# jdwapman/essentials

Hardware: NVIDIA B200
Metric: BFS GTEPS (higher is better)
Workload: dtype int32

## Files before the change

### essentials_b200/csrc/capi_core.cu

```cuda
#include "capi_common.hxx"
#include <algorithm>
#include <memory>
#include <gunrock/algorithms/generate/random.hxx>
#include <gunrock/algorithms/sssp.hxx>

namespace ess {
std::string& last_error() {
  static thread_local std::string message;
  return message;
}
int fail(const std::exception& e) {
  last_error() = e.what();
  return 999;
}
int fail(const char* message, int code) {
  last_error() = message;
  return code;
}
}

using namespace gunrock;

namespace ess {
int& dist_peer_exchange() {
  static int on = 1;
  return on;
}
int& dist_trace() {
  static int on = 0;
  return on;
}
int& dist_peer_timeout_ms() {
  static int ms = 4000;
  return ms;
}
int& host_chunk_edges() {
  static int edges = 64 << 20;
  return edges;
}
}

extern "C" {

const char* ess_last_error(void) { return ess::last_error().c_str(); }
int ess_version(void) { return 100; }

int ess_context_create(int device, void* stream, int own_stream, ess_context_t* out) {
  ESS_TRY
  if (!out) return ess::fail("ess_context_create: out is null");
  int count = 0;
  error::throw_if_exception(cudaGetDeviceCount(&count), "no CUDA device");
  error::throw_if_exception(device < 0 || device >= count, "ess_context_create: bad device ordinal");
  auto* h = new ess_context_s;
  if (own_stream)
    h->ctx = std::make_shared<gcuda::multi_context_t>(device);
  else
    h->ctx = std::make_shared<gcuda::multi_context_t>(device, static_cast<cudaStream_t>(stream));
  h->single()->scratch();
  *out = h;
  return 0;
  ESS_CATCH
}

int ess_context_destroy(ess_context_t ctx) {
  delete ctx;
  return 0;
}

int ess_context_synchronize(ess_context_t ctx) {
  ESS_TRY
  ctx->single()->synchronize();
  return 0;
  ESS_CATCH
}

int ess_tune(const char* knob, int value) {
  ESS_TRY
  const std::string k = knob ? knob : "";
  if (k == "near_far_ctas") {
    gunrock::operators::advance::near_far_ctas_per_sm() = value < 1 ? 1 : value;
    return 0;
  }
  if (k == "advance_engine") {
    gunrock::operators::advance::kernels::advance_engine() = value;
    return 0;
  }
  if (k == "pull_engine") {
    gunrock::operators::advance::kernels::pull_engine() = value;
    return 0;
  }
  if (k == "near_far_cluster") {
    gunrock::operators::advance::near_far_cluster_enabled() = value;
    return 0;
  }
  if (k == "pull_hints") {
    gunrock::operators::advance::kernels::pull_hints_enabled() = value;
    return 0;
  }
  if (k == "sssp_fused_unique") {
    gunrock::sssp::fused_unique() = value;
    return 0;
  }
  if (k == "dist_trace") {
    ess::dist_trace() = value;
    return 0;
  }
  if (k == "dist_peer_exchange") {
    ess::dist_peer_exchange() = value;
    return 0;
  }
  if (k == "host_chunk_edges") {
    if (value <= 0) return ess::fail("ess_tune: host_chunk_edges must be positive");
    ess::host_chunk_edges() = value;
    return 0;
  }
  if (k == "dist_peer_timeout_ms") {
    if (value <= 0) return ess::fail("ess_tune: dist_peer_timeout_ms must be positive");
    ess::dist_peer_timeout_ms() = value;
    return 0;
  }
  return ess::fail("ess_tune: unknown knob");
  ESS_CATCH
}

int ess_profile_enable(ess_context_t ctx, int enable) {
  ESS_TRY
  auto& prof = ctx->single()->profiler();
  prof.reset();
  prof.enabled = enable != 0;
  return 0;
  ESS_CATCH
}

int ess_profile_read(ess_context_t ctx, double* ms_by_class, int64_t* launches_by_class, int n_classes) {
  ESS_TRY
  auto& prof = ctx->single()->profiler();
  prof.collect();
  for (int i = 0; i < n_classes && i < gcuda::profiler_t::n_classes; ++i) {
    if (ms_by_class) ms_by_class[i] = prof.ms[i];
    if (launches_by_class) launches_by_class[i] = prof.launches[i];
  }
  if (launches_by_class && n_classes >= gcuda::profiler_t::n_classes)
    launches_by_class[gcuda::profiler_t::n_classes - 1] = prof.launches_total;
  return 0;
  ESS_CATCH
}

int ess_graph_create(int64_t n, int64_t m, int offset_bits, const void* d_row_offsets,
                     const int32_t* d_column_indices, const float* d_values, int symmetric,
                     const void* d_column_offsets, const int32_t* d_row_indices, const float* d_csc_values,
                     ess_graph_t* out) {
  ESS_TRY
  if (!out || !d_row_offsets || (m > 0 && !d_column_indices)) return ess::fail("ess_graph_create: null argument");
  if (offset_bits != 32 && offset_bits != 64) return ess::fail("ess_graph_create: offset_bits must be 32 or 64");
  if (n < 0 || n > 2147483647LL) return ess::fail("ess_graph_create: vertex ids are int32");
  if (offset_bits == 32 && m > 2147483647LL) return ess::fail("ess_graph_create: m needs 64-bit offsets");
  auto* h = new ess_graph_s;
  h->offset_bits = offset_bits;
  h->n = n;
  h->m = m;
  const void* t_off = d_column_offsets;
  const int32_t* t_idx = d_row_indices;
  const float* t_val = d_csc_values;
  if (symmetric) {
    t_off = d_row_offsets;
    t_idx = d_column_indices;
    t_val = d_values;
  }
  h->has_csc = t_off != nullptr;
  auto* J = const_cast<int32_t*>(d_column_indices);
  auto* X = const_cast<float*>(d_values);
  auto* I = const_cast<int32_t*>(t_idx);
  auto* Xt = const_cast<float*>(t_val);
  if (offset_bits == 64)
    h->g64 = graph::build::from_csr_and_csc<int32_t, int64_t, float>(
        int32_t(n), int64_t(m), (int64_t*)d_row_offsets, J, X, (int64_t*)t_off, I, Xt);
  else
    h->g32 = graph::build::from_csr_and_csc<int32_t, int32_t, float>(
        int32_t(n), int32_t(m), (int32_t*)d_row_offsets, J, X, (int32_t*)t_off, I, Xt);
  if (h->has_csc && symmetric != 2 && n > 0 && m > 0) {
    int rc = ess_graph_build_pull_hints(h, nullptr);
    if (rc) {
      delete h;
      return rc;
    }
  }
  *out = h;
  return 0;
  ESS_CATCH
}

}

namespace {
struct copy_lane_t {
  cudaStream_t stream = nullptr;
  std::vector<cudaEvent_t> events;
  copy_lane_t() { error::throw_if_exception(cudaStreamCreateWithFlags(&stream, cudaStreamNonBlocking), "copy stream"); }
  ~copy_lane_t() {
    for (auto e : events) cudaEventDestroy(e);
    if (stream) cudaStreamDestroy(stream);
  }
  void publish_to(cudaStream_t follower) {
    cudaEvent_t e = nullptr;
    error::throw_if_exception(cudaEventCreateWithFlags(&e, cudaEventDisableTiming), "copy event");
    events.push_back(e);
    error::throw_if_exception(cudaEventRecord(e, stream), "copy event record");
    error::throw_if_exception(cudaStreamWaitEvent(follower, e, 0), "copy event wait");
  }
};

template <typename edge_t>
void create_from_host(ess_context_t ctx, ess_graph_s* h, const void* h_row_offsets, const int32_t* h_column_indices,
                      const float* h_values, bool symmetric) {
  auto* c = ctx->single();
  cudaStream_t work = c->stream();
  const std::size_t n = std::size_t(h->n), m = std::size_t(h->m);
  const edge_t* ho = static_cast<const edge_t*>(h_row_offsets);
  error::throw_if_exception(ho[0] != edge_t(0) || std::size_t(ho[n]) != m,
                            "ess_graph_create_from_host: row_offsets[0] must be 0 and row_offsets[n] must be m");
  h->own_offsets.resize((n + 1) * sizeof(edge_t));
  h->own_indices.resize(m);
  if (h_values) h->own_values.resize(m);
  edge_t* d_off = reinterpret_cast<edge_t*>(h->own_offsets.data());
  int32_t* d_idx = h->own_indices.data();
  float* d_val = h_values ? h->own_values.data() : nullptr;

  copy_lane_t lane;
  error::throw_if_exception(cudaMemcpyAsync(d_off, ho, (n + 1) * sizeof(edge_t), cudaMemcpyHostToDevice, lane.stream),
                            "ess_graph_create_from_host: offsets copy");
  lane.publish_to(work);
  const bool hints = symmetric && n > 0 && m > 0;
  memory::device_array_t<int32_t> degree;
  edge_t* hint_edge = nullptr;
  if (hints) {
    h->hint_head.resize(n);
    h->hint_isolated.resize((n + 31) / 32 + 1);
    if constexpr (sizeof(edge_t) == 8) {
      h->hint_edge64.resize(n);
      hint_edge = h->hint_edge64.data();
    } else {
      h->hint_edge32.resize(n);
      hint_edge = h->hint_edge32.data();
    }
    degree.resize(n);
    graph::build::detail::degrees_kernel<<<2048, 256, 0, work>>>(int32_t(n), d_off, degree.data());
    graph::build::detail::isolated_bitmap_kernel<<<2048, 256, 0, work>>>(int32_t(n), d_off, h->hint_isolated.data());
  }
  const std::size_t chunk_edges = std::size_t(ess::host_chunk_edges());
  std::size_t built = 0;
  for (std::size_t e0 = 0; e0 < m; e0 += chunk_edges) {
    const std::size_t e1 = std::min(m, e0 + chunk_edges);
    error::throw_if_exception(cudaMemcpyAsync(d_idx + e0, h_column_indices + e0, (e1 - e0) * sizeof(int32_t),
                                              cudaMemcpyHostToDevice, lane.stream),
                              "ess_graph_create_from_host: indices copy");
    if (!hints) continue;
    lane.publish_to(work);
    const std::size_t arrived = std::size_t(std::upper_bound(ho, ho + n + 1, edge_t(e1)) - ho) - 1;
    graph::build::pull_hints_range(int32_t(built), int32_t(arrived), d_off, d_idx, degree.data(), h->hint_head.data(),
                                   hint_edge, work);
    built = std::max(built, arrived);
  }
  if (d_val)
    error::throw_if_exception(cudaMemcpyAsync(d_val, h_values, m * sizeof(float), cudaMemcpyHostToDevice, lane.stream),
                              "ess_graph_create_from_host: values copy");
  error::throw_if_exception(cudaStreamSynchronize(lane.stream), "ess_graph_create_from_host: copy");
  error::throw_if_exception(cudaStreamSynchronize(work), "ess_graph_create_from_host: hint build");
  error::check_last("ess_graph_create_from_host");

  auto G = graph::build::from_csr_and_csc<int32_t, edge_t, float>(int32_t(n), edge_t(m), d_off, d_idx, d_val,
                                                                  symmetric ? d_off : nullptr,
                                                                  symmetric ? d_idx : nullptr,
                                                                  symmetric ? d_val : nullptr);
  if (hints) {
    graph::graph_csc_t<int32_t, edge_t, float>& csc = G;
    csc.set_pull_hints(h->hint_head.data(), hint_edge, h->hint_isolated.data());
  }
  if constexpr (sizeof(edge_t) == 8)
    h->g64 = G;
  else
    h->g32 = G;
}
}

extern "C" {

int ess_graph_create_from_host(ess_context_t ctx, int64_t n, int64_t m, int offset_bits, const void* h_row_offsets,
                               const int32_t* h_column_indices, const float* h_values, int symmetric,
                               ess_graph_t* out) {
  ESS_TRY
  if (!ctx || !out || !h_row_offsets || (m > 0 && !h_column_indices))
    return ess::fail("ess_graph_create_from_host: null argument");
  if (offset_bits != 32 && offset_bits != 64)
    return ess::fail("ess_graph_create_from_host: offset_bits must be 32 or 64");
  if (n < 0 || n > 2147483647LL) return ess::fail("ess_graph_create_from_host: vertex ids are int32");
  if (m < 0 || (offset_bits == 32 && m > 2147483647LL))
    return ess::fail("ess_graph_create_from_host: m needs 64-bit offsets");
  std::unique_ptr<ess_graph_s> h(new ess_graph_s);
  h->offset_bits = offset_bits;
  h->n = n;
  h->m = m;
  h->has_csc = symmetric != 0;
  if (offset_bits == 64)
    create_from_host<int64_t>(ctx, h.get(), h_row_offsets, h_column_indices, h_values, symmetric != 0);
  else
    create_from_host<int32_t>(ctx, h.get(), h_row_offsets, h_column_indices, h_values, symmetric != 0);
  *out = h.release();
  return 0;
  ESS_CATCH
}

int ess_graph_build_pull_hints(ess_graph_t h, const int32_t* d_degree_of_id) {
  ESS_TRY
  if (!h || !h->has_csc) return ess::fail("ess_graph_build_pull_hints: graph has no CSC view");
  if (h->n <= 0 || h->m <= 0) return 0;
  error::throw_if_exception(cudaDeviceSynchronize(), "ess_graph_build_pull_hints: pending work failed");
  h->hint_head.resize(std::size_t(h->n));
  h->hint_isolated.resize((std::size_t(h->n) + 31) / 32 + 1);
  if (h->offset_bits == 64) {
    h->hint_edge64.resize(std::size_t(h->n));
    graph::build::pull_hints(h->g64, h->hint_head.data(), h->hint_edge64.data(), 0, d_degree_of_id,
                             h->hint_isolated.data());
  } else {
    h->hint_edge32.resize(std::size_t(h->n));
    graph::build::pull_hints(h->g32, h->hint_head.data(), h->hint_edge32.data(), 0, d_degree_of_id,
                             h->hint_isolated.data());
  }
  return 0;
  ESS_CATCH
}

int ess_graph_destroy(ess_graph_t g) {
  delete g;
  return 0;
}

int ess_transpose_csr(int64_t n, int64_t m, int offset_bits, const void* d_row_offsets,
                      const int32_t* d_column_indices, const float* d_values, void* d_out_offsets,
                      int32_t* d_out_indices, float* d_out_values) {
  ESS_TRY
  error::throw_if_exception(cudaDeviceSynchronize(), "ess_transpose_csr: pending work failed");
  if (offset_bits == 64)
    graph::build::detail::transpose_on_device<int32_t, int64_t, float>(
        int32_t(n), int64_t(m), (const int64_t*)d_row_offsets, d_column_indices, d_values, d_out_indices,
        (int64_t*)d_out_offsets, d_out_values);
  else
    graph::build::detail::transpose_on_device<int32_t, int32_t, float>(
        int32_t(n), int32_t(m), (const int32_t*)d_row_offsets, d_column_indices, d_values, d_out_indices,
        (int32_t*)d_out_offsets, d_out_values);
  return 0;
  ESS_CATCH
}

int ess_randoms(ess_context_t ctx, float* d_out, int64_t n, float begin, float end) {
  ESS_TRY
  generate::random::uniform_distribution(d_out, std::size_t(n), begin, end, ctx->single()->stream());
  error::check_last("ess_randoms");
  ctx->single()->synchronize();
  return 0;
  ESS_CATCH
}

int ess_frontier_to_bitmap(ess_context_t ctx, const int32_t* d_list, int64_t size, int64_t universe,
                           uint32_t* d_words, int64_t* popcount) {
  ESS_TRY
  auto* c = ctx->single();
  auto stream = c->stream();
  auto& scratch = c->scratch();
  const std::size_t words = (std::size_t(universe) + 31) / 32;
  cudaMemsetAsync(d_words, 0, words * sizeof(uint32_t), stream);
  if (size)
    frontier::kernels::scatter_bits_kernel<<<gcuda::persistent_grid(*c, (std::size_t(size) + 255) / 256, 8), 256, 0,
                                             stream>>>(d_list, std::size_t(size), d_words);
  scratch.zero(stream);
  frontier::kernels::popcount_kernel<<<gcuda::persistent_grid(*c, (words + 255) / 256, 8), 256, 0, stream>>>(
      d_words, words, scratch.d + gcuda::scratch_t::out_count);
  error::check_last("ess_frontier_to_bitmap");
  scratch.fetch(stream);
  if (popcount) *popcount = int64_t(scratch.h[gcuda::scratch_t::out_count]);
  return 0;
  ESS_CATCH
}

int ess_bitmap_to_frontier(ess_context_t ctx, const uint32_t* d_words, int64_t universe, int32_t* d_list,
                           int64_t* out_count) {
  ESS_TRY
  auto* c = ctx->single();
  auto stream = c->stream();
  auto& scratch = c->scratch();
  const std::size_t words = (std::size_t(universe) + 31) / 32;
  scratch.zero(stream);
  frontier::kernels::gather_bits_kernel<<<gcuda::persistent_grid(*c, (words + 255) / 256, 8), 256, 0, stream>>>(
      d_words, words, d_list, scratch.d + gcuda::scratch_t::out_count);
  error::check_last("ess_bitmap_to_frontier");
  scratch.fetch(stream);
  if (out_count) *out_count = int64_t(scratch.h[gcuda::scratch_t::out_count]);
  return 0;
  ESS_CATCH
}

int ess_bits_to_list_async(ess_context_t ctx, const uint32_t* d_words, int64_t universe, int32_t* d_list) {
  ESS_TRY
  auto* c = ctx->single();
  auto stream = c->stream();
  auto& scratch = c->scratch();
  const std::size_t words = (std::size_t(universe) + 31) / 32;
  scratch.zero(stream);
  frontier::kernels::gather_bits_kernel<<<gcuda::persistent_grid(*c, (words + 255) / 256, 8), 256, 0, stream>>>(
      d_words, words, d_list, scratch.d + gcuda::scratch_t::out_count);
  error::check_last("ess_bits_to_list_async");
  return 0;
  ESS_CATCH
}

}
```

### include/gunrock/framework/operators/advance/kernels.cuh

```cuda
#pragma once

#include <gunrock/b200/warp.cuh>
#include <gunrock/b200/lookback.cuh>
#include <gunrock/framework/operators/advance/directional.cuh>
#include <gunrock/cuda/context.hxx>
#include <gunrock/graph/graph.hxx>
#include <gunrock/util/type_limits.hxx>

namespace gunrock {
namespace operators {
namespace advance {
namespace kernels {

using b200::counter_t;
using gcuda::scratch_t;

constexpr int cta_threads = 256;
constexpr int tile_items = 4;
constexpr int tile_edges = cta_threads * tile_items;
constexpr int prep_items = 4;
constexpr long long big_degree = 4096;
constexpr int warp_degree = 32;

enum class visit_t { none, test_and_set, unique_output };

constexpr bool count_fresh_edges_in_kernel = false;

template <visit_t policy, typename vertex_t, typename edge_t, typename weight_t, typename operator_t>
__device__ __forceinline__ bool visit_edge(const graph::adjacency_t<vertex_t, edge_t, weight_t>& A,
                                           operator_t& op, vertex_t source, edge_t edge, vertex_t neighbor,
                                           unsigned* __restrict__ visited, counter_t& fresh_edges) {
  if constexpr (policy == visit_t::test_and_set) {
    if ((visited[unsigned(neighbor) >> 5] >> (unsigned(neighbor) & 31u)) & 1u) return false;
  }
  weight_t weight = A.values ? __ldg(A.values + edge) : weight_t(1);
  source += A.source_offset;
  bool keep = op(source, neighbor, edge, weight);
  if constexpr (policy == visit_t::test_and_set) {
    if (keep) {
      const unsigned bit = 1u << (unsigned(neighbor) & 31u);
      keep = !(atomicOr(&visited[unsigned(neighbor) >> 5], bit) & bit);
      if constexpr (count_fresh_edges_in_kernel)
        if (keep) fresh_edges += counter_t(A.offsets[neighbor + 1] - A.offsets[neighbor]);
    }
  }
  if constexpr (policy == visit_t::unique_output) {
    if (keep) {
      const unsigned bit = 1u << (unsigned(neighbor) & 31u);
      unsigned* word = &visited[unsigned(neighbor) >> 5];
      keep = !(*word & bit) && !(atomicOr(word, bit) & bit);
    }
  }
  return keep;
}

template <typename vertex_t>
__global__ void __launch_bounds__(256)
    clear_emitted_kernel(const vertex_t* __restrict__ output, std::size_t count, unsigned* __restrict__ seen) {
  for (std::size_t i = std::size_t(blockIdx.x) * blockDim.x + threadIdx.x; i < count;
       i += std::size_t(gridDim.x) * blockDim.x) {
    const vertex_t v = output[i];
    if (util::limits::is_valid(v)) seen[unsigned(v) >> 5] = 0u;
  }
}

template <visit_t policy>
__device__ __forceinline__ void flush_fresh_edges(counter_t fresh_edges, counter_t* counters) {
  if constexpr (policy == visit_t::test_and_set && count_fresh_edges_in_kernel) {
    __syncwarp();
    fresh_edges = b200::warp_sum(fresh_edges);
    if (b200::lane_id() == 0 && fresh_edges) atomicAdd(counters + scratch_t::aux2, fresh_edges);
  }
}

template <typename vertex_t, typename edge_t>
struct tile_smem_t {
  vertex_t src[tile_edges + 1];
  edge_t beg[tile_edges + 1];
  edge_t seg[tile_edges + 1];
  counter_t append[cta_threads / 32 + 4];
  edge_t scan_e[cta_threads / 32 + 1];
  unsigned scan_u[cta_threads / 32 + 1];
  long long bcast[4];
};

template <bool has_output, visit_t policy, typename vertex_t, typename edge_t, typename weight_t, typename operator_t>
__device__ __forceinline__ void expand_tile(const graph::adjacency_t<vertex_t, edge_t, weight_t>& A, operator_t& op,
                                            tile_smem_t<vertex_t, edge_t>& sm, int n_seg, edge_t n_edges,
                                            vertex_t* __restrict__ output, counter_t* counters, counter_t capacity,
                                            unsigned* __restrict__ visited, counter_t& fresh_edges,
                                            edge_t edge_base = 0) {
  for (edge_t round = 0; round < n_edges; round += tile_edges) {
    vertex_t nbr[tile_items];
    vertex_t src[tile_items];
    edge_t eid[tile_items];
    unsigned live = 0;
#pragma unroll
    for (int i = 0; i < tile_items; ++i) {
      edge_t r = round + edge_t(i * cta_threads + threadIdx.x);
      if (r < n_edges) {
        const edge_t at = r + edge_base;
        int j = n_seg == 1 ? 0 : b200::upper_segment(sm.seg, n_seg, at);
        src[i] = sm.src[j];
        eid[i] = sm.beg[j] + (at - sm.seg[j]);
        live |= 1u << i;
      }
    }
#pragma unroll
    for (int i = 0; i < tile_items; ++i)
      if (live & (1u << i)) nbr[i] = __ldg(A.indices + eid[i]);
    unsigned keep = 0;
    if constexpr (policy == visit_t::test_and_set && has_pull_operator<operator_t>::value) {
      unsigned word[tile_items], old[tile_items];
#pragma unroll
      for (int i = 0; i < tile_items; ++i)
        if (live & (1u << i)) word[i] = visited[unsigned(nbr[i]) >> 5];
#pragma unroll
      for (int i = 0; i < tile_items; ++i)
        if ((live & (1u << i)) && ((word[i] >> (unsigned(nbr[i]) & 31u)) & 1u)) live &= ~(1u << i);
#pragma unroll
      for (int i = 0; i < tile_items; ++i)
        if (live & (1u << i)) old[i] = atomicOr(&visited[unsigned(nbr[i]) >> 5], 1u << (unsigned(nbr[i]) & 31u));
#pragma unroll
      for (int i = 0; i < tile_items; ++i)
        if ((live & (1u << i)) && !((old[i] >> (unsigned(nbr[i]) & 31u)) & 1u)) {
          const weight_t weight = A.values ? __ldg(A.values + eid[i]) : weight_t(1);
          if (call_pull(op, vertex_t(src[i] + A.source_offset), nbr[i], eid[i], weight)) keep |= 1u << i;
        }
      if constexpr (count_fresh_edges_in_kernel) {
        edge_t lo[tile_items], hi[tile_items];
#pragma unroll
        for (int i = 0; i < tile_items; ++i)
          if (keep & (1u << i)) {
            lo[i] = A.offsets[nbr[i]];
            hi[i] = A.offsets[nbr[i] + 1];
          }
#pragma unroll
        for (int i = 0; i < tile_items; ++i)
          if (keep & (1u << i)) fresh_edges += counter_t(hi[i] - lo[i]);
      }
    } else {
#pragma unroll
      for (int i = 0; i < tile_items; ++i)
        if (live & (1u << i))
          if (visit_edge<policy>(A, op, src[i], eid[i], nbr[i], visited, fresh_edges)) keep |= 1u << i;
    }
    if constexpr (has_output)
      b200::cta_append<cta_threads, tile_items>(nbr, keep, output, counters + scratch_t::out_count, capacity,
                                                sm.append);
  }
}

__device__ __forceinline__ bool output_fits(counter_t* counters, counter_t capacity) {
  const counter_t worst = counters[scratch_t::work_total];
  if (worst <= capacity) return true;
  if (blockIdx.x == 0 && threadIdx.x == 0) counters[scratch_t::overflow] = worst;
  return false;
}

template <bool graph_input, typename vertex_t, typename edge_t>
__global__ void __launch_bounds__(cta_threads)
    degree_sum_kernel(const edge_t* __restrict__ offsets, const vertex_t* __restrict__ input, std::size_t input_size,
                      counter_t* counters) {
  counter_t mine = 0;
  for (std::size_t i = std::size_t(blockIdx.x) * cta_threads + threadIdx.x; i < input_size;
       i += std::size_t(gridDim.x) * cta_threads) {
    vertex_t v = graph_input ? vertex_t(i) : input[i];
    if (util::limits::is_valid(v)) mine += counter_t(offsets[v + 1] - offsets[v]);
  }
  mine = b200::warp_sum(mine);
  if (b200::lane_id() == 0 && mine) atomicAdd(counters + scratch_t::work_total, mine);
}

template <typename vertex_t, typename edge_t>
__global__ void __launch_bounds__(cta_threads)
    max_degree_kernel(const edge_t* __restrict__ offsets, vertex_t n, counter_t* result) {
  counter_t mine = 0;
  for (std::size_t v = std::size_t(blockIdx.x) * cta_threads + threadIdx.x; v < std::size_t(n);
       v += std::size_t(gridDim.x) * cta_threads) {
    counter_t d = counter_t(offsets[v + 1] - offsets[v]);
    mine = d > mine ? d : mine;
  }
  mine = b200::warp_max(mine);
  if (b200::lane_id() == 0) atomicMax(result, mine);
}

template <bool graph_input, bool has_output, bool guard, visit_t policy, typename vertex_t, typename edge_t,
          typename weight_t, typename operator_t>
__global__ void __launch_bounds__(cta_threads)
    thread_mapped_kernel(const graph::adjacency_t<vertex_t, edge_t, weight_t> A, operator_t op,
                         const vertex_t* __restrict__ input, std::size_t input_size, const counter_t* size_ptr,
                         vertex_t* __restrict__ output, counter_t* counters, counter_t capacity,
                         unsigned* __restrict__ visited) {
  if constexpr (has_output && guard)
    if (!output_fits(counters, capacity)) return;
  if (size_ptr) input_size = std::size_t(*size_ptr);
  counter_t fresh_edges = 0;
  for (std::size_t base = std::size_t(blockIdx.x) * cta_threads; base < input_size;
       base += std::size_t(gridDim.x) * cta_threads) {
    const std::size_t i = base + threadIdx.x;
    vertex_t v = gunrock::numeric_limits<vertex_t>::invalid();
    edge_t beg = 0, deg = 0;
    if (i < input_size) {
      v = graph_input ? vertex_t(i) : input[i];
      if (util::limits::is_valid(v)) {
        beg = A.offsets[v];
        deg = A.offsets[v + 1] - beg;
      }
    }
    const edge_t trips = b200::warp_max(deg);
    for (edge_t k = 0; k < trips; ++k) {
      bool keep = false;
      vertex_t nbr = 0;
      if (k < deg) {
        nbr = __ldg(A.indices + beg + k);
        keep = visit_edge<policy>(A, op, v, edge_t(beg + k), nbr, visited, fresh_edges);
      }
      if constexpr (has_output) {
        const unsigned votes = __ballot_sync(b200::full_mask, keep);
        if (votes) {
          counter_t at = b200::warp_append_slot(keep, counters + scratch_t::out_count);
          if (keep && at < capacity) output[at] = nbr;
        }
      }
    }
  }
  flush_fresh_edges<policy>(fresh_edges, counters);
}

template <bool has_output, visit_t policy, typename vertex_t, typename edge_t, typename weight_t, typename operator_t>
__global__ void __launch_bounds__(cta_threads)
    warp_mapped_kernel(const graph::adjacency_t<vertex_t, edge_t, weight_t> A, operator_t op,
                       const vertex_t* __restrict__ list, const counter_t* size_ptr, vertex_t* __restrict__ output,
                       counter_t* counters, counter_t capacity, unsigned* __restrict__ visited) {
  if constexpr (has_output)
    if (!output_fits(counters, capacity)) return;
  const std::size_t count = std::size_t(*size_ptr);
  const unsigned lane = b200::lane_id();
  const std::size_t warps = (std::size_t(gridDim.x) * cta_threads) >> 5;
  counter_t fresh_edges = 0;
  for (std::size_t item = (std::size_t(blockIdx.x) * cta_threads + threadIdx.x) >> 5; item < count; item += warps) {
    vertex_t v = list[item];
    const edge_t beg = A.offsets[v], end = A.offsets[v + 1];
    for (edge_t e0 = beg; e0 < end; e0 += 32) {
      const edge_t e = e0 + lane;
      bool keep = false;
      vertex_t nbr = 0;
      if (e < end) {
        nbr = __ldg(A.indices + e);
        keep = visit_edge<policy>(A, op, v, e, nbr, visited, fresh_edges);
      }
      if constexpr (has_output) {
        const unsigned votes = __ballot_sync(b200::full_mask, keep);
        if (votes) {
          counter_t at = b200::warp_append_slot(keep, counters + scratch_t::out_count);
          if (keep && at < capacity) output[at] = nbr;
        }
      }
    }
  }
  flush_fresh_edges<policy>(fresh_edges, counters);
}

template <bool graph_input, bool has_output, bool guard, visit_t policy, typename vertex_t, typename edge_t,
          typename weight_t, typename operator_t>
__global__ void __launch_bounds__(cta_threads)
    block_mapped_kernel(const graph::adjacency_t<vertex_t, edge_t, weight_t> A, operator_t op,
                        const vertex_t* __restrict__ input, std::size_t input_size, vertex_t* __restrict__ output,
                        counter_t* counters, counter_t capacity, unsigned* __restrict__ visited,
                        vertex_t* __restrict__ big_list) {
  __shared__ tile_smem_t<vertex_t, edge_t> sm;
  if constexpr (has_output && guard)
    if (!output_fits(counters, capacity)) return;
  counter_t fresh_edges = 0;
  for (std::size_t base = std::size_t(blockIdx.x) * cta_threads; base < input_size;
       base += std::size_t(gridDim.x) * cta_threads) {
    const std::size_t i = base + threadIdx.x;
    vertex_t v = gunrock::numeric_limits<vertex_t>::invalid();
    edge_t beg = 0, deg = 0;
    if (i < input_size) {
      v = graph_input ? vertex_t(i) : input[i];
      if (util::limits::is_valid(v)) {
        beg = A.offsets[v];
        deg = A.offsets[v + 1] - beg;
      }
    }
    if (big_list && deg >= edge_t(big_degree)) {
      counter_t at = atomicAdd(counters + scratch_t::big_count, counter_t(1));
      big_list[at] = v;
      deg = 0;
    }
    unsigned n_seg;
    edge_t n_edges;
    const unsigned my_seg = b200::cta_exclusive_sum<cta_threads, unsigned>(deg > 0 ? 1u : 0u, n_seg, sm.scan_u);
    const edge_t my_off = b200::cta_exclusive_sum<cta_threads, edge_t>(deg, n_edges, sm.scan_e);
    if (deg > 0) {
      sm.src[my_seg] = v;
      sm.beg[my_seg] = beg;
      sm.seg[my_seg] = my_off;
    }
    __syncthreads();
    if (n_edges > 0)
      expand_tile<has_output, policy>(A, op, sm, int(n_seg), n_edges, output, counters, capacity, visited,
                                      fresh_edges);
    __syncthreads();
  }
  flush_fresh_edges<policy>(fresh_edges, counters);
}

template <bool has_output, visit_t policy, typename vertex_t, typename edge_t, typename weight_t, typename operator_t>
__global__ void __launch_bounds__(cta_threads)
    big_list_kernel(const graph::adjacency_t<vertex_t, edge_t, weight_t> A, operator_t op,
                    const vertex_t* __restrict__ big_list, const counter_t* size_ptr, vertex_t* __restrict__ output,
                    counter_t* counters, counter_t capacity, unsigned* __restrict__ visited) {
  __shared__ tile_smem_t<vertex_t, edge_t> sm;
  if constexpr (has_output)
    if (!output_fits(counters, capacity)) return;
  const std::size_t count = std::size_t(*size_ptr);
  counter_t fresh_edges = 0;
  for (std::size_t item = 0; item < count; ++item) {
    const vertex_t v = big_list[item];
    const edge_t beg = A.offsets[v], deg = A.offsets[v + 1] - beg;
    for (edge_t t0 = edge_t(blockIdx.x) * tile_edges; t0 < deg; t0 += edge_t(gridDim.x) * tile_edges) {
      if (threadIdx.x == 0) {
        sm.src[0] = v;
        sm.beg[0] = beg + t0;
        sm.seg[0] = 0;
      }
      __syncthreads();
      const edge_t left = deg - t0;
      expand_tile<has_output, policy>(A, op, sm, 1, left < edge_t(tile_edges) ? left : edge_t(tile_edges), output,
                                      counters, capacity, visited, fresh_edges);
      __syncthreads();
    }
  }
  flush_fresh_edges<policy>(fresh_edges, counters);
}

template <bool graph_input, typename vertex_t, typename edge_t>
__global__ void __launch_bounds__(cta_threads)
    prepare_work_kernel(const edge_t* __restrict__ offsets, const vertex_t* __restrict__ input, std::size_t input_size,
                        vertex_t* __restrict__ work_src, edge_t* __restrict__ work_beg, edge_t* __restrict__ work_seg,
                        b200::tile_word_t* state_items, b200::tile_word_t* state_edges, counter_t* counters) {
  constexpr int per_tile = cta_threads * prep_items;
  __shared__ unsigned scan_u[cta_threads / 32 + 1];
  __shared__ unsigned long long scan_e[cta_threads / 32 + 1];
  __shared__ unsigned long long prefix[2];
  __shared__ int s_tile;
  const int n_tiles = int((input_size + per_tile - 1) / per_tile);
  const bool vector_input = (reinterpret_cast<std::uintptr_t>(input) & 15u) == 0;
  for (;;) {
    if (threadIdx.x == 0) s_tile = int(atomicAdd(counters + scratch_t::ticket, counter_t(1)));
    __syncthreads();
    const int tile = s_tile;
    if (tile >= n_tiles) break;
    const std::size_t first = std::size_t(tile) * per_tile + std::size_t(threadIdx.x) * prep_items;
    vertex_t v[prep_items];
    edge_t beg[prep_items], deg[prep_items];
    if constexpr (!graph_input) {
      if (vector_input && first + prep_items <= input_size && prep_items == 4 && sizeof(vertex_t) == 4) {
        const int4 q = *reinterpret_cast<const int4*>(input + first);
        v[0] = vertex_t(q.x), v[1] = vertex_t(q.y), v[2] = vertex_t(q.z), v[3] = vertex_t(q.w);
      } else {
#pragma unroll
        for (int k = 0; k < prep_items; ++k)
          v[k] = first + k < input_size ? input[first + k] : gunrock::numeric_limits<vertex_t>::invalid();
      }
    } else {
#pragma unroll
      for (int k = 0; k < prep_items; ++k)
        v[k] = first + k < input_size ? vertex_t(first + k) : gunrock::numeric_limits<vertex_t>::invalid();
    }
    unsigned my_items = 0;
    unsigned long long my_edges = 0;
#pragma unroll
    for (int k = 0; k < prep_items; ++k) {
      beg[k] = 0, deg[k] = 0;
      if (util::limits::is_valid(v[k])) {
        beg[k] = offsets[v[k]];
        deg[k] = offsets[v[k] + 1] - beg[k];
      }
      my_items += deg[k] > 0;
      my_edges += (unsigned long long)deg[k];
    }
    unsigned tile_items_total;
    unsigned long long tile_edges_total;
    const unsigned items_before = b200::cta_exclusive_sum<cta_threads, unsigned>(my_items, tile_items_total, scan_u);
    const unsigned long long edges_before =
        b200::cta_exclusive_sum<cta_threads, unsigned long long>(my_edges, tile_edges_total, scan_e);
    if (threadIdx.x < 32) {
      const unsigned long long a = b200::lookback_exclusive(state_items, tile, tile_items_total);
      const unsigned long long b = b200::lookback_exclusive(state_edges, tile, tile_edges_total);
      if (threadIdx.x == 0) {
        prefix[0] = a;
        prefix[1] = b;
      }
    }
    __syncthreads();
    std::size_t at = std::size_t(prefix[0]) + items_before;
    unsigned long long run = prefix[1] + edges_before;
#pragma unroll
    for (int k = 0; k < prep_items; ++k)
      if (deg[k] > 0) {
        work_src[at] = v[k];
        work_beg[at] = beg[k];
        work_seg[at] = edge_t(run);
        ++at;
        run += (unsigned long long)deg[k];
      }
    if (tile == n_tiles - 1 && threadIdx.x == 0) {
      const unsigned long long K = prefix[0] + tile_items_total, T = prefix[1] + tile_edges_total;
      counters[scratch_t::items] = K;
      counters[scratch_t::work_total] = T;
      work_seg[K] = edge_t(T);
    }
    __syncthreads();
  }
}

template <bool has_output, visit_t policy, typename vertex_t, typename edge_t, typename weight_t, typename operator_t>
__global__ void __launch_bounds__(cta_threads)
    merge_path_kernel(const graph::adjacency_t<vertex_t, edge_t, weight_t> A, operator_t op,
                      const vertex_t* __restrict__ work_src, const edge_t* __restrict__ work_beg,
                      const edge_t* __restrict__ work_seg, vertex_t* __restrict__ output, counter_t* counters,
                      counter_t capacity, unsigned* __restrict__ visited) {
  __shared__ tile_smem_t<vertex_t, edge_t> sm;
  if constexpr (has_output)
    if (!output_fits(counters, capacity)) return;
  const long long total = (long long)counters[scratch_t::work_total];
  const long long n_items = (long long)counters[scratch_t::items];
  counter_t fresh_edges = 0;
  const long long n_tiles = (total + tile_edges - 1) / tile_edges;
  const long long per_cta = (n_tiles + gridDim.x - 1) / gridDim.x;
  const long long first_tile = (long long)blockIdx.x * per_cta;
  const long long last_tile = first_tile + per_cta < n_tiles ? first_tile + per_cta : n_tiles;
  long long j0 = 0;
  for (long long tile = first_tile; tile < last_tile; ++tile) {
    const long long g0 = tile * tile_edges;
    const long long g1 = g0 + tile_edges < total ? g0 + tile_edges : total;
    if (tile == first_tile) {
      if (threadIdx.x == 0) {
        long long lo = 0, hi = n_items;
        while (hi - lo > 1) {
          const long long mid = (lo + hi) >> 1;
          if ((long long)work_seg[mid] <= g0)
            lo = mid;
          else
            hi = mid;
        }
        sm.bcast[0] = lo;
      }
      __syncthreads();
      j0 = sm.bcast[0];
    }
    int n_seg = 0;
    {
      unsigned mine = 0;
      for (int j = threadIdx.x; j <= tile_edges; j += cta_threads) {
        const long long jj = j0 + j;
        if (jj < n_items) {
          const long long s = (long long)work_seg[jj];
          if (s < g1) {
            sm.src[j] = work_src[jj];
            sm.beg[j] = work_beg[jj] + edge_t(s < g0 ? g0 - s : 0);
            sm.seg[j] = edge_t(s < g0 ? 0 : s - g0);
            ++mine;
          }
        }
      }
      unsigned total_seg;
      b200::cta_exclusive_sum<cta_threads, unsigned>(mine, total_seg, sm.scan_u);
      n_seg = int(total_seg);
    }
    __syncthreads();
    expand_tile<has_output, policy>(A, op, sm, n_seg, edge_t(g1 - g0), output, counters, capacity, visited,
                                    fresh_edges);
    {
      const long long last = j0 + n_seg - 1;
      const long long last_end = (long long)work_seg[last + 1];
      j0 = last_end > g1 ? last : last + 1;
    }
    __syncthreads();
  }
  flush_fresh_edges<policy>(fresh_edges, counters);
}

template <bool graph_input, bool has_output, visit_t policy, typename vertex_t, typename edge_t, typename weight_t,
          typename operator_t>
__global__ void __launch_bounds__(cta_threads)
    merge_path_small_kernel(const graph::adjacency_t<vertex_t, edge_t, weight_t> A, operator_t op,
                            const vertex_t* __restrict__ input, int input_size, vertex_t* __restrict__ output,
                            counter_t* counters, counter_t capacity, unsigned* __restrict__ visited) {
  __shared__ tile_smem_t<vertex_t, edge_t> sm;
  vertex_t v[tile_items];
  edge_t beg[tile_items], deg[tile_items];
  unsigned my_items = 0;
  edge_t my_edges = 0;
#pragma unroll
  for (int k = 0; k < tile_items; ++k) {
    const int i = int(threadIdx.x) * tile_items + k;
    v[k] = gunrock::numeric_limits<vertex_t>::invalid();
    beg[k] = deg[k] = 0;
    if (i < input_size) {
      v[k] = graph_input ? vertex_t(i) : input[i];
      if (util::limits::is_valid(v[k])) {
        beg[k] = A.offsets[v[k]];
        deg[k] = A.offsets[v[k] + 1] - beg[k];
      }
    }
    my_items += deg[k] > 0;
    my_edges += deg[k];
  }
  unsigned n_seg;
  edge_t total;
  unsigned at = b200::cta_exclusive_sum<cta_threads, unsigned>(my_items, n_seg, sm.scan_u);
  edge_t run = b200::cta_exclusive_sum<cta_threads, edge_t>(my_edges, total, sm.scan_e);
#pragma unroll
  for (int k = 0; k < tile_items; ++k)
    if (deg[k] > 0) {
      sm.src[at] = v[k];
      sm.beg[at] = beg[k];
      sm.seg[at] = run;
      ++at;
      run += deg[k];
    }
  __syncthreads();
  if (blockIdx.x == 0 && threadIdx.x == 0) counters[scratch_t::work_total] = counter_t(total);
  if constexpr (has_output) {
    if (counter_t(total) > capacity) {
      if (blockIdx.x == 0 && threadIdx.x == 0) counters[scratch_t::overflow] = counter_t(total);
      return;
    }
  }
  counter_t fresh_edges = 0;
  for (edge_t g0 = edge_t(blockIdx.x) * tile_edges; g0 < total; g0 += edge_t(gridDim.x) * tile_edges) {
    const edge_t left = total - g0;
    expand_tile<has_output, policy>(A, op, sm, int(n_seg), left < edge_t(tile_edges) ? left : edge_t(tile_edges),
                                    output, counters, capacity, visited, fresh_edges, g0);
  }
  flush_fresh_edges<policy>(fresh_edges, counters);
}

template <bool graph_input, typename vertex_t, typename edge_t>
__global__ void __launch_bounds__(cta_threads)
    bin_by_degree_kernel(const edge_t* __restrict__ offsets, const vertex_t* __restrict__ input,
                         std::size_t input_size, vertex_t* __restrict__ small_list, vertex_t* __restrict__ warp_list,
                         vertex_t* __restrict__ big_list, counter_t* counters) {
  counter_t my_edges = 0;
  for (std::size_t base = std::size_t(blockIdx.x) * cta_threads; base < input_size;
       base += std::size_t(gridDim.x) * cta_threads) {
    const std::size_t i = base + threadIdx.x;
    edge_t deg = 0;
    vertex_t v = 0;
    if (i < input_size) {
      v = graph_input ? vertex_t(i) : input[i];
      if (util::limits::is_valid(v)) deg = offsets[v + 1] - offsets[v];
    }
    my_edges += counter_t(deg);
    const bool is_big = deg >= edge_t(big_degree);
    const bool is_warp = !is_big && deg >= edge_t(warp_degree);
    const bool is_small = deg > 0 && deg < edge_t(warp_degree);
    if (__ballot_sync(b200::full_mask, is_small)) {
      counter_t at = b200::warp_append_slot(is_small, counters + scratch_t::aux0);
      if (is_small) small_list[at] = v;
    }
    if (__ballot_sync(b200::full_mask, is_warp)) {
      counter_t at = b200::warp_append_slot(is_warp, counters + scratch_t::aux1);
      if (is_warp) warp_list[at] = v;
    }
    if (__ballot_sync(b200::full_mask, is_big)) {
      counter_t at = b200::warp_append_slot(is_big, counters + scratch_t::big_count);
      if (is_big) big_list[at] = v;
    }
  }
  my_edges = b200::warp_sum(my_edges);
  if (b200::lane_id() == 0 && my_edges) atomicAdd(counters + scratch_t::work_total, my_edges);
}

}
}
}
}
```

### include/gunrock/framework/operators/advance/pull.cuh

```cuda
#pragma once

#include <type_traits>
#include <utility>
#include <gunrock/b200/warp.cuh>
#include <gunrock/framework/operators/advance/directional.cuh>
#include <gunrock/cuda/context.hxx>
#include <gunrock/graph/graph.hxx>

namespace gunrock {
namespace operators {
namespace advance {
namespace kernels {

using b200::counter_t;
using gcuda::scratch_t;

template <typename vertex_t>
__device__ __forceinline__ vertex_t hint_vertex(vertex_t h) { return h < -1 ? vertex_t(-2) - h : h; }

template <typename vertex_t, typename edge_t>
__global__ void __launch_bounds__(256)
    init_visited_kernel(const edge_t* __restrict__ offsets, vertex_t n, unsigned* __restrict__ visited) {
  const unsigned lane = b200::lane_id();
  const std::size_t n_words = (std::size_t(n) + 31) / 32;
  const std::size_t warps = (std::size_t(gridDim.x) * blockDim.x) >> 5;
  for (std::size_t w = (std::size_t(blockIdx.x) * blockDim.x + threadIdx.x) >> 5; w < n_words; w += warps) {
    const std::size_t v = w * 32 + lane;
    bool skip = true;
    if (v < std::size_t(n)) skip = offsets[v + 1] == offsets[v];
    const unsigned word = __ballot_sync(b200::full_mask, skip);
    if (lane == 0) visited[w] = word;
  }
}

template <typename vertex_t, typename edge_t>
__global__ void __launch_bounds__(256)
    mark_frontier_kernel(const edge_t* __restrict__ offsets, const vertex_t* __restrict__ list, std::size_t count,
                         const counter_t* count_ptr, unsigned* __restrict__ visited, counter_t* counters) {
  if (count_ptr) count = std::size_t(*count_ptr);
  counter_t mine = 0;
  for (std::size_t i = std::size_t(blockIdx.x) * blockDim.x + threadIdx.x; i < count;
       i += std::size_t(gridDim.x) * blockDim.x) {
    const vertex_t v = list[i];
    if (!util::limits::is_valid(v)) continue;
    if (visited) atomicOr(&visited[unsigned(v) >> 5], 1u << (unsigned(v) & 31u));
    mine += counter_t(offsets[v + 1] - offsets[v]);
  }
  __syncwarp();
  mine = b200::warp_sum(mine);
  if (b200::lane_id() == 0 && mine) atomicAdd(counters + scratch_t::aux2, mine);
}

template <typename vertex_t, typename edge_t, typename weight_t, typename operator_t>
__global__ void __launch_bounds__(256, 6)
    pull_step_kernel(const graph::adjacency_t<vertex_t, edge_t, weight_t> A, operator_t op,
                     const unsigned* __restrict__ frontier_bits, unsigned* __restrict__ next_bits,
                     unsigned* __restrict__ visited, counter_t* counters) {
  const unsigned lane = b200::lane_id();
  const unsigned n = unsigned(A.n);
  const unsigned n_words = (n + 31u) >> 5;
  const unsigned warps = (gridDim.x * blockDim.x) >> 5;
  const bool hinted = A.head != nullptr;
  unsigned found_vertices = 0, scanned = 0, inspected = 0;
  counter_t found_edges = 0;

  struct stage_t {
    unsigned seen;
    edge_t beg, end;
    vertex_t head;
  };
  auto load_seen = [&](unsigned w) -> unsigned { return w < n_words ? visited[w] : 0xffffffffu; };
  auto load_stage = [&](unsigned w, unsigned seen) {
    stage_t s{seen, 0, 0, vertex_t(-1)};
    if (!((seen >> lane) & 1u)) {
      const unsigned v = (w << 5) + lane;
      s.beg = A.offsets[v];
      s.end = A.offsets[v + 1];
      if (hinted) s.head = hint_vertex(__ldg(A.head + v));
    }
    return s;
  };
  auto probe_of = [&](const stage_t& s) -> unsigned {
    return s.head >= 0 ? __ldg(frontier_bits + (unsigned(s.head) >> 5)) : 0u;
  };

  unsigned w = (blockIdx.x * blockDim.x + threadIdx.x) >> 5;
  stage_t cur = load_stage(w, load_seen(w));
  stage_t nxt = load_stage(w + warps, load_seen(w + warps));
  unsigned seen_far = load_seen(w + 2 * warps);
  unsigned probe = probe_of(cur);
  while (w < n_words) {
    const unsigned seen_farther = load_seen(w + 3 * warps);
    const stage_t far = load_stage(w + 2 * warps, seen_far);
    const unsigned probe_next = probe_of(nxt);
    bool found = false;
    if (!((cur.seen >> lane) & 1u)) {
      ++scanned;
      const vertex_t v = vertex_t((w << 5) + lane);
      bool head_tried = false;
      if (cur.head >= 0 && ((probe >> (unsigned(cur.head) & 31u)) & 1u)) {
        const edge_t edge = __ldg(A.head_edge + v);
        const weight_t weight = A.values ? __ldg(A.values + edge) : weight_t(1);
        found = call_pull(op, cur.head, v, edge, weight);
        head_tried = true;
      }
      for (edge_t e = cur.beg; e < cur.end && !found; ++e) {
        ++inspected;
        const vertex_t u = __ldg(A.indices + e);
        if (head_tried && u == cur.head) continue;
        if ((__ldg(frontier_bits + (unsigned(u) >> 5)) >> (unsigned(u) & 31u)) & 1u) {
          const weight_t weight = A.values ? __ldg(A.values + e) : weight_t(1);
          found = call_pull(op, u, v, e, weight);
        }
      }
    }
    const unsigned fresh = __ballot_sync(b200::full_mask, found);
    if (lane == 0) {
      next_bits[w] = fresh;
      if (fresh) visited[w] = cur.seen | fresh;
      found_vertices += __popc(fresh);
    }
    if (found) found_edges += counter_t(cur.end - cur.beg);
    w += warps;
    cur = nxt;
    nxt = far;
    seen_far = seen_farther;
    probe = probe_next;
  }
  found_edges = b200::warp_sum(found_edges);
  scanned = b200::warp_sum(scanned);
  inspected = b200::warp_sum(inspected);
  if (lane == 0) {
    if (found_vertices) atomicAdd(counters + scratch_t::out_count, counter_t(found_vertices));
    if (found_edges) atomicAdd(counters + scratch_t::aux2, found_edges);
    if (scanned) atomicAdd(counters + scratch_t::aux0, counter_t(scanned));
    if (inspected) atomicAdd(counters + scratch_t::aux1, counter_t(inspected));
  }
}

constexpr int pull_chunk_words = 32;
constexpr int pull_queue_cap = 32 + 4 * 32;
constexpr int pull_long_list = 64;

template <typename vertex_t, typename edge_t, typename weight_t, typename operator_t>
__global__ void __launch_bounds__(256, 5)
    pull_chunk_kernel(const graph::adjacency_t<vertex_t, edge_t, weight_t> A, operator_t op,
                      const unsigned* __restrict__ frontier_bits, unsigned* __restrict__ next_bits,
                      unsigned* __restrict__ visited, counter_t* counters) {
  __shared__ unsigned short s_open[8][pull_chunk_words * 32];
  __shared__ unsigned s_queue[8][pull_queue_cap];
  __shared__ unsigned s_fresh[8][pull_chunk_words];
  const unsigned lane = b200::lane_id();
  unsigned short* open_list = s_open[b200::warp_id()];
  unsigned* queue = s_queue[b200::warp_id()];
  unsigned* fresh_words = s_fresh[b200::warp_id()];
  const unsigned n = unsigned(A.n);
  const unsigned n_words = (n + 31u) >> 5;
  const unsigned n_chunks = (n_words + pull_chunk_words - 1) / pull_chunk_words;
  const unsigned warps = (gridDim.x * blockDim.x) >> 5;
  const bool hinted = A.head != nullptr;
  unsigned found_vertices = 0, scanned = 0, inspected = 0, walked = 0;
  unsigned queued = 0;
  unsigned live_chunk = 0xffffffffu;
  constexpr unsigned tried_flag = 0x80000000u;

  auto drain = [&](unsigned take) {
    unsigned entry = 0;
    const bool mine = lane < take;
    if (mine) entry = queue[queued - take + lane];
    queued -= take;
    const bool head_tried = (entry & tried_flag) != 0;
    const vertex_t v = vertex_t(entry & ~tried_flag);
    edge_t beg = 0, end = 0;
    if (mine) {
      beg = A.offsets[v];
      end = A.offsets[v + 1];
      ++walked;
    }
    const vertex_t head = (mine && head_tried) ? hint_vertex(__ldg(A.head + v)) : vertex_t(-1);
    bool found = false;
    const bool is_long = mine && (end - beg) > edge_t(pull_long_list);
    if (mine && !is_long) {
      for (edge_t e = beg; e < end && !found; ++e) {
        ++inspected;
        const vertex_t u = __ldg(A.indices + e);
        if (u == head) continue;
        if ((__ldg(frontier_bits + (unsigned(u) >> 5)) >> (unsigned(u) & 31u)) & 1u) {
          const weight_t weight = A.values ? __ldg(A.values + e) : weight_t(1);
          found = call_pull(op, u, v, e, weight);
        }
      }
    }
    unsigned long_lanes = __ballot_sync(b200::full_mask, is_long);
    while (long_lanes) {
      const int owner = __ffs(long_lanes) - 1;
      long_lanes &= long_lanes - 1;
      const vertex_t ov = __shfl_sync(b200::full_mask, v, owner);
      const vertex_t ohead = __shfl_sync(b200::full_mask, head, owner);
      const edge_t ob = __shfl_sync(b200::full_mask, beg, owner);
      const edge_t oe = __shfl_sync(b200::full_mask, end, owner);
      bool done = false;
      for (edge_t e0 = ob; e0 < oe && !done; e0 += 32) {
        const edge_t e = e0 + edge_t(lane);
        vertex_t u = vertex_t(-1);
        bool candidate = false;
        if (e < oe) {
          ++inspected;
          u = __ldg(A.indices + e);
          candidate = u != ohead && ((__ldg(frontier_bits + (unsigned(u) >> 5)) >> (unsigned(u) & 31u)) & 1u);
        }
        unsigned votes = __ballot_sync(b200::full_mask, candidate);
        while (votes && !done) {
          const int first = __ffs(votes) - 1;
          votes &= votes - 1;
          bool ok = false;
          if (int(lane) == first) {
            const weight_t weight = A.values ? __ldg(A.values + e) : weight_t(1);
            ok = call_pull(op, u, ov, e, weight);
          }
          done = __shfl_sync(b200::full_mask, ok, first);
        }
      }
      if (int(lane) == owner) found = done;
    }
    if (found) {
      const unsigned bit = 1u << (unsigned(v) & 31u);
      if ((unsigned(v) >> 10) == live_chunk) {
        atomicOr(fresh_words + ((unsigned(v) >> 5) & 31u), bit);
      } else {
        atomicOr(next_bits + (unsigned(v) >> 5), bit);
        atomicOr(visited + (unsigned(v) >> 5), bit);
        ++found_vertices;
      }
    }
    __syncwarp();
  };

  for (unsigned chunk = (blockIdx.x * blockDim.x + threadIdx.x) >> 5; chunk < n_chunks; chunk += warps) {
    const unsigned w_mine = chunk * pull_chunk_words + lane;
    const unsigned seen_mine = w_mine < n_words ? visited[w_mine] : 0xffffffffu;
    fresh_words[lane] = 0u;
    live_chunk = chunk;
    unsigned open_bits = ~seen_mine;
    const unsigned mine_open = __popc(open_bits);
    const unsigned incl = b200::warp_inclusive_sum(mine_open);
    const unsigned total = __shfl_sync(b200::full_mask, incl, 31);
    {
      unsigned at = incl - mine_open;
      while (open_bits) {
        const unsigned b = __ffs(open_bits) - 1;
        open_bits &= open_bits - 1;
        open_list[at++] = (unsigned short)((lane << 5) | b);
      }
    }
    __syncwarp();
    if (lane == 0) scanned += total;
    for (unsigned base = 0; base < total; base += 128) {
      unsigned loc[4];
      vertex_t hid[4];
      bool single[4];
      unsigned probe[4];
#pragma unroll
      for (int k = 0; k < 4; ++k) {
        const unsigned idx = base + 32u * k + lane;
        loc[k] = idx < total ? unsigned(open_list[idx]) : 0xffffffffu;
        vertex_t h = vertex_t(-1);
        if (loc[k] != 0xffffffffu && hinted) h = __ldg(A.head + ((chunk << 10) + loc[k]));
        single[k] = h < vertex_t(-1);
        hid[k] = hint_vertex(h);
      }
#pragma unroll
      for (int k = 0; k < 4; ++k) probe[k] = hid[k] >= 0 ? __ldg(frontier_bits + (unsigned(hid[k]) >> 5)) : 0u;
#pragma unroll
      for (int k = 0; k < 4; ++k) {
        const bool valid = loc[k] != 0xffffffffu;
        const vertex_t v = vertex_t((chunk << 10) + (valid ? loc[k] : 0u));
        bool found = false, tried = false;
        if (valid && hid[k] >= 0 && ((probe[k] >> (unsigned(hid[k]) & 31u)) & 1u)) {
          const edge_t edge = __ldg(A.head_edge + v);
          const weight_t weight = A.values ? __ldg(A.values + edge) : weight_t(1);
          found = call_pull(op, hid[k], v, edge, weight);
          tried = true;
        }
        if (found) atomicOr(fresh_words + (loc[k] >> 5), 1u << (loc[k] & 31u));
        const bool miss = valid && !found && !(single[k] && hinted);
        const unsigned misses = __ballot_sync(b200::full_mask, miss);
        if (miss) queue[queued + __popc(misses & b200::lanes_below(lane))] = unsigned(v) | (tried ? tried_flag : 0u);
        queued += __popc(misses);
      }
      __syncwarp();
      while (queued >= 32) drain(32);
    }
    __syncwarp();
    const unsigned fresh_mine = fresh_words[lane];
    if (w_mine < n_words) {
      next_bits[w_mine] = fresh_mine;
      if (fresh_mine) visited[w_mine] = seen_mine | fresh_mine;
    }
    found_vertices += __popc(fresh_mine);
    live_chunk = 0xffffffffu;
    __syncwarp();
  }
  if (queued) drain(queued);

  found_vertices = b200::warp_sum(found_vertices);
  scanned = b200::warp_sum(scanned);
  inspected = b200::warp_sum(inspected);
  walked = b200::warp_sum(walked);
  if (lane == 0) {
    if (found_vertices) atomicAdd(counters + scratch_t::out_count, counter_t(found_vertices));
    if (scanned) atomicAdd(counters + scratch_t::aux0, counter_t(scanned));
    if (inspected) atomicAdd(counters + scratch_t::aux1, counter_t(inspected));
    if (walked) atomicAdd(counters + scratch_t::aux2, counter_t(walked));
  }
}

inline int& pull_engine() {
  static int engine = 1;
  return engine;
}

inline int& pull_hints_enabled() {
  static int enabled = 1;
  return enabled;
}

}
}
}
}
```

Measured before the change: 2002.

## Reconstruct BFS depths from per-level visited bitmap snapshots and use pull operator on push visits

Adds a kernel that rebuilds per-vertex BFS depths from stored per-level visited bitmaps. It counts, for each vertex, how many snapshots have its bit set, using byte-packed SWAR counting, then writes the depths through a shared-memory transpose with 128-bit stores. This is meant to remove per-edge depth writes during traversal. The push test-and-set path also now claims the visited bit with atomicOr before calling the pull-style operator, when the operator provides one. The snapshot mode is exposed as a tune knob. The BFS algorithm file that would allocate snapshots and launch the kernel is not part of this change, so it is unclear whether the new path runs.

Measured after the change: 2054, median of 6. 1.03x the previous value.

```diff
diff --git a/essentials_b200/csrc/capi_core.cu b/essentials_b200/csrc/capi_core.cu
--- a/essentials_b200/csrc/capi_core.cu
+++ b/essentials_b200/csrc/capi_core.cu
@@ -1,6 +1,7 @@
 #include "capi_common.hxx"
 #include <algorithm>
 #include <memory>
+#include <gunrock/algorithms/bfs.hxx>
 #include <gunrock/algorithms/generate/random.hxx>
 #include <gunrock/algorithms/sssp.hxx>
 
@@ -95,6 +96,11 @@
   }
   if (k == "pull_hints") {
     gunrock::operators::advance::kernels::pull_hints_enabled() = value;
+    return 0;
+  }
+  if (k == "bfs_depth_snapshots") {
+    if (value < 0 || value > 255) return ess::fail("ess_tune: bfs_depth_snapshots must be in 0..255");
+    gunrock::bfs::depth_snapshots() = value;
     return 0;
   }
   if (k == "sssp_fused_unique") {
diff --git a/include/gunrock/framework/operators/advance/kernels.cuh b/include/gunrock/framework/operators/advance/kernels.cuh
--- a/include/gunrock/framework/operators/advance/kernels.cuh
+++ b/include/gunrock/framework/operators/advance/kernels.cuh
@@ -30,6 +30,16 @@
 __device__ __forceinline__ bool visit_edge(const graph::adjacency_t<vertex_t, edge_t, weight_t>& A,
                                            operator_t& op, vertex_t source, edge_t edge, vertex_t neighbor,
                                            unsigned* __restrict__ visited, counter_t& fresh_edges) {
+  if constexpr (policy == visit_t::test_and_set && has_pull_operator<operator_t>::value) {
+    const unsigned bit = 1u << (unsigned(neighbor) & 31u);
+    unsigned* word = &visited[unsigned(neighbor) >> 5];
+    if ((*word & bit) || (atomicOr(word, bit) & bit)) return false;
+    const weight_t weight = A.values ? __ldg(A.values + edge) : weight_t(1);
+    const bool keep = call_pull(op, vertex_t(source + A.source_offset), neighbor, edge, weight);
+    if constexpr (count_fresh_edges_in_kernel)
+      if (keep) fresh_edges += counter_t(A.offsets[neighbor + 1] - A.offsets[neighbor]);
+    return keep;
+  }
   if constexpr (policy == visit_t::test_and_set) {
     if ((visited[unsigned(neighbor) >> 5] >> (unsigned(neighbor) & 31u)) & 1u) return false;
   }
diff --git a/include/gunrock/framework/operators/advance/pull.cuh b/include/gunrock/framework/operators/advance/pull.cuh
--- a/include/gunrock/framework/operators/advance/pull.cuh
+++ b/include/gunrock/framework/operators/advance/pull.cuh
@@ -1,5 +1,7 @@
 #pragma once
 
+#include <cstdint>
+#include <limits>
 #include <type_traits>
 #include <utility>
 #include <gunrock/b200/warp.cuh>
@@ -49,6 +51,75 @@
   __syncwarp();
   mine = b200::warp_sum(mine);
   if (b200::lane_id() == 0 && mine) atomicAdd(counters + scratch_t::aux2, mine);
+}
+
+template <typename vertex_t, typename edge_t>
+__global__ void __launch_bounds__(256)
+    depth_from_snapshots_kernel(vertex_t* __restrict__ depth, vertex_t n, vertex_t source,
+                                const unsigned* __restrict__ snapshots, std::size_t stride, int levels,
+                                const unsigned* __restrict__ isolated, const edge_t* __restrict__ in_offsets) {
+  static_assert(sizeof(vertex_t) == 4, "depths are staged and stored as 128-bit groups of four");
+  constexpr vertex_t unreached = std::numeric_limits<vertex_t>::max();
+  constexpr int row = 36;
+  __shared__ __align__(16) vertex_t s_depth[8][32 * row];
+  vertex_t* tile = s_depth[b200::warp_id()];
+  const unsigned lane = b200::lane_id();
+  const bool vector_store = (reinterpret_cast<std::uintptr_t>(depth) & 15u) == 0;
+  const std::size_t n_words = (std::size_t(n) + 31) / 32;
+  const std::size_t n_chunks = (n_words + 31) / 32;
+  const std::size_t warps = (std::size_t(gridDim.x) * blockDim.x) >> 5;
+  for (std::size_t chunk = (std::size_t(blockIdx.x) * blockDim.x + threadIdx.x) >> 5; chunk < n_chunks;
+       chunk += warps) {
+    const std::size_t w = chunk * 32 + lane;
+    const std::size_t wl = w < n_words ? w : n_words - 1;
+    const unsigned no_in = isolated ? __ldg(isolated + wl) : 0u;
+    unsigned held[8] = {0, 0, 0, 0, 0, 0, 0, 0};
+    for (int k0 = 0; k0 < levels; k0 += 8) {
+      unsigned word[8];
+#pragma unroll
+      for (int j = 0; j < 8; ++j) word[j] = __ldg(snapshots + std::size_t(min(k0 + j, levels - 1)) * stride + wl);
+#pragma unroll
+      for (int j = 0; j < 8; ++j)
+        if (k0 + j < levels)
+#pragma unroll
+          for (int q = 0; q < 8; ++q)
+            held[q] += (((word[j] >> (4 * q)) & 0xfu) * 0x00204081u) & 0x01010101u;
+    }
+#pragma unroll
+    for (int q = 0; q < 8; ++q) {
+      vertex_t d[4];
+#pragma unroll
+      for (int i = 0; i < 4; ++i) {
+        const int b = 4 * q + i;
+        const std::size_t v = w * 32 + b;
+        const int h = int((held[q] >> (8 * i)) & 0xffu);
+        d[i] = h ? vertex_t(levels + 1 - h) : unreached;
+        if (h && h == levels) {
+          const bool none =
+              isolated ? ((no_in >> b) & 1u) != 0 : (v < std::size_t(n) && in_offsets[v + 1] == in_offsets[v]);
+          if (none) d[i] = unreached;
+        }
+        if (v == std::size_t(source)) d[i] = vertex_t(0);
+      }
+      *reinterpret_cast<int4*>(tile + lane * row + 4 * q) = make_int4(int(d[0]), int(d[1]), int(d[2]), int(d[3]));
+    }
+    __syncwarp();
+#pragma unroll
+    for (int t = 0; t < 8; ++t) {
+      const unsigned g = unsigned(t) * 32u + lane;
+      const int4 d4 = *reinterpret_cast<const int4*>(tile + (g >> 3) * row + 4 * (g & 7u));
+      const std::size_t v0 = chunk * 1024 + std::size_t(g) * 4;
+      if (vector_store && v0 + 4 <= std::size_t(n)) {
+        *reinterpret_cast<int4*>(depth + v0) = d4;
+      } else {
+        const int d[4] = {d4.x, d4.y, d4.z, d4.w};
+#pragma unroll
+        for (int i = 0; i < 4; ++i)
+          if (v0 + i < std::size_t(n)) depth[v0 + i] = vertex_t(d[i]);
+      }
+    }
+    __syncwarp();
+  }
 }
 
 template <typename vertex_t, typename edge_t, typename weight_t, typename operator_t>
```
